# ChalmersPhotonicsLab/QAMpy

Hardware: AMD Instinct MI355X
Metric: equalised MSym/s (2-pol, 2 SPS) (higher is better)
Workload: dtype f32

## Files before the change

### qampy_amd/csrc/api.hip

```cpp
#include "common.h"
#include <stdlib.h>
#include <atomic>
#include <mutex>
#include <vector>
#include <unordered_map>
#include <string.h>

namespace qh {

thread_local hipStream_t g_stream = nullptr;
static thread_local hipStream_t g_streams[4] = {nullptr, nullptr, nullptr, nullptr};
int g_device = -1;
static thread_local std::string g_err;
static std::mutex g_mu;

void set_error(const std::string &s) { g_err = s; }

int hip_fail(hipError_t e, const char *what, const char *file, int line)
{
    g_err = std::string(hipGetErrorString(e)) + " in " + what + " (" + file + ":" + std::to_string(line) + ")";
    (void)hipGetLastError();
    return QH_ERR_HIP;
}

// ... 71 lines not shown
hipStream_t helper_stream() { return g_streams[3]; }

int ensure_init()
{
    if (g_stream) return QH_OK;
    return init_device(g_device >= 0 ? g_device : 0);
}

thread_local void *g_scratch[SCRATCH_SLOTS] = {nullptr};
thread_local size_t g_scratch_n[SCRATCH_SLOTS] = {0};
thread_local unsigned g_scratch_epoch = 0;
static std::atomic<int> g_form[FORM_COUNT];
struct FormName { const char *key, *env; };
static const FormName FORM_NAMES[FORM_COUNT] = {
    {"trainer", "QAMPY_HIP_TRAINER"}, {"pit_form", "QAMPY_HIP_PIT_FORM"}, {"seg_lanes", "QAMPY_HIP_SEG_LANES"}, {"pit_probe", "QAMPY_HIP_PIT_PROBE"},
    {"bps", "QAMPY_HIP_BPS"}, {"pit_tail", "QAMPY_HIP_PIT_TAIL"}};
static int form_parse(int k, const char *v, int *out)
{
    if (!v || !v[0]) { *out = 0; return 0; }
    switch (k) {
    case FORM_TRAINER: *out = v[0] == 'd' ? 1 : (v[0] == 'l' ? 2 : (v[0] == 'i' ? 3 : (v[0] == 'a' || v[0] == '0' ? 0 : -1))); break;
    case FORM_PIT: *out = v[0] == 's' ? 1 : (v[0] == 'b' ? 2 : (v[0] == 'a' || v[0] == '0' ? 0 : -1)); break;
    case FORM_SEG_LANES: { const int n = atoi(v); *out = (n == 8 || n == 16 || n == 0) ? n : -1; break; }
    case FORM_BPS: *out = v[0] == 't' ? 1 : (v[0] == 'l' ? 2 : (v[0] == 'a' || v[0] == '0' ? 0 : -1)); break;
    case FORM_PIT_TAIL: *out = v[0] == 's' ? 1 : (v[0] == 'a' || v[0] == '0' ? 0 : -1); break;
    default: *out = atoi(v) != 0 ? 1 : 0; break;
    }
    return *out < 0 ? -1 : 0;
}
static const int g_form_env_read = [] {
    for (int k = 0; k < FORM_COUNT; k++) {
        int v = 0;
        if (form_parse(k, getenv(FORM_NAMES[k].env), &v) == 0) g_form[k].store(v);
    }
    return 0;
}();
int form(FormKey k) { return g_form[k].load(std::memory_order_relaxed); }
const char *trainer_force()
{
    switch (form(FORM_TRAINER)) {
// ... 378 lines not shown
```

### qampy_amd/csrc/common.h

```cpp
#pragma once
#include <hip/hip_runtime.h>
#include <stdint.h>
#include <string>
#include "../../include/qampy_hip.h"

namespace qh {

extern thread_local hipStream_t g_stream;
extern int g_device;
void set_error(const std::string &s);
int hip_fail(hipError_t e, const char *what, const char *file, int line);

#define QH_HIP(call)                                                        \
    do {                                                                    \
        hipError_t _e = (call);                                             \
        if (_e != hipSuccess) return qh::hip_fail(_e, #call, __FILE__, __LINE__); \
    } while (0)

#define QH_REQUIRE(cond, msg)                                   \
    do {                                                        \
        if (!(cond)) { qh::set_error(msg); return QH_ERR_ARG; } \
    } while (0)

#define QH_WAVE_FIRST() __builtin_amdgcn_s_setprio(3)

int ensure_init();
hipStream_t side_stream();
hipStream_t helper_stream();
enum FormKey { FORM_TRAINER = 0, FORM_PIT, FORM_SEG_LANES, FORM_PIT_PROBE, FORM_BPS, FORM_PIT_TAIL, FORM_COUNT };
int form(FormKey k);
const char *trainer_force();
double gram_budget_gb();
int pit_timing_mode();
int default_tier();
double default_tier_tol();
constexpr int SCRATCH_SLOTS = 28;
constexpr int SCRATCH_TWOSTAGE = 16;
constexpr int SCRATCH_FOE = 17;
constexpr int SCRATCH_IMPAIR = 18;
constexpr int SCRATCH_PMD = 19;
constexpr int SCRATCH_TXRESP = 20;
constexpr int SCRATCH_SOS = 21;
constexpr int SCRATCH_CPR = 22;
constexpr int SCRATCH_FFT = 23;
// ... 173 lines not shown
```

### qampy_amd/csrc/train_pit.h

```cpp
#pragma once
#include <atomic>
#include <chrono>
#include <vector>
#include "train_impl.h"
#include "train_seg.h"

namespace qh {

typedef qh_pit_report PitCtrl;

constexpr double PIT_CONTRACT = 0.2;
constexpr int PIT_PROBE = 128;
constexpr int PIT_SEEDWIN = 512;
constexpr int PIT_MAXSEG = 65536;

__host__ __device__ inline int pit_symmetry(int method)
{
    switch (method) {
    case QH_M_CMA: case QH_M_SGNCMA: case QH_M_RDE: return 0;
    case QH_M_CMA2: return 2;
    default: return 4;
    }
}

// ... 34 lines not shown
    __syncthreads();
    return r;
}

template <typename T> __device__ __forceinline__ void block_prefix_sum(T *a, int n, T *tot)
{
    const int len = (n + 255) / 256;
    const int i0 = threadIdx.x * len, i1 = i0 + len < n ? i0 + len : n;
    T s = 0;
    for (int i = i0; i < i1; i++) s += a[i];
    T run = block_scan_excl<T>(s, [](T x, T y) { return x + y; }, (T)0, tot);
    for (int i = i0; i < i1; i++) { run += a[i]; a[i] = run; }
    __syncthreads();
}

template <typename R>
__global__ void __launch_bounds__(256) pit_setup_kernel(const Cx<R> *E, int nmodes, int64_t L, int64_t npow, int ntot, const R *mu, double gear,
                                                        double bound, double tol, PitSeg sg, PitCtrl *c, R *mu_acq)
{
    QH_WAVE_FIRST();
    __shared__ double red[256];
    double acc = 0;
    for (int k = 0; k < nmodes; k++)
        for (int64_t i = threadIdx.x; i < npow; i += 256) {
            const Cx<R> v = E[(size_t)k * L + i];
            acc += (double)v.re * v.re + (double)v.im * v.im;
        }
    red[threadIdx.x] = acc;
    __syncthreads();
    for (int s = 128; s > 0; s >>= 1) {
        if (threadIdx.x < s) red[threadIdx.x] += red[threadIdx.x + s];
        __syncthreads();
    }
    if (threadIdx.x == 0) {
        const double p = red[0] / ((double)nmodes * (double)npow);
        const double m = (double)*mu;
        double ma = gear * m;
        const double cap = bound / ((double)ntot * (p > 1e-30 ? p : 1e-30));
        if (ma > cap) ma = cap;
        if (!(ma > m)) ma = m;
        c->segments = sg.S; c->seg_len = sg.len; c->mu = m; c->mu_acq = ma; c->power = p; c->tol = tol;
        for (int q = 0; q < QH_PIT_MAXPASS; q++) { c->result_change[q] = -1; c->deviation[q] = -1; c->deviation_rms[q] = -1; c->deviation_taps[q] = -1; c->deviation_taps_worst[q] = -1; } c->passes = 0; c->converged = 0; c->acq_chunks = 0; c->acq_steps = 0; c->acq_done = 0; c->done = 0; c->diverged = 0; c->corr_on = 0; c->gain = 0; c->out_power = 0;
        for (int i = 0; i < QH_PIT_MAXPASS; i++) c->defect[i] = -1;
        for (int i = 0; i < QH_PIT_MAXCHUNK; i++) c->acq_err[i] = -1;
        *mu_acq = (R)ma;
    }
}

template <typename R>
__global__ void __launch_bounds__(256) pit_acq_monitor_kernel(const Cx<R> *err, int64_t err_pitch, int64_t step0, int64_t n, int nsel,
                                                              const int64_t *modes_dev, double plateau, PitCtrl *c, R *mu_acq, const R *mu, double floor_gear)
{
    QH_WAVE_FIRST();
    if (threadIdx.x == 0 && floor_gear >= 0) {
        const R lo = (R)((double)*mu * floor_gear), h = *mu_acq * (R)0.5;
        *mu_acq = h > lo ? h : (*mu_acq > lo ? lo : *mu_acq);
    }
    if (c->acq_done) return;
    __shared__ double red[256];
    double acc = 0;
// ... 72 lines not shown
            }
        }
        const double y2r = (double)yr * yr - (double)yi * yi, y2i = 2.0 * yr * yi;
        zr += y2r * y2r - y2i * y2i;
        zi += 2.0 * y2r * y2i;
    }
    rr[threadIdx.x] = zr; ri[threadIdx.x] = zi;
    __syncthreads();
    for (int q = 128; q > 0; q >>= 1) {
        if (threadIdx.x < q) { rr[threadIdx.x] += rr[threadIdx.x + q]; ri[threadIdx.x] += ri[threadIdx.x + q]; }
        __syncthreads();
    }
    if (threadIdx.x == 0) { z[2 * ((size_t)s * gridDim.y + j)] = rr[0]; z[2 * ((size_t)s * gridDim.y + j) + 1] = ri[0]; }
}

static __global__ void __launch_bounds__(256) pit_unwrap_kernel(const double *z, int S, int nsel, double *rot, double *phi, int *jump)
{
    QH_WAVE_FIRST();
    __shared__ int ptot[512];
    const double q = 1.5707963267948966;
    phi += (size_t)blockIdx.x * S; jump += (size_t)blockIdx.x * S;
    for (int j = blockIdx.x; j <= (int)blockIdx.x; j++) {
        for (int s = threadIdx.x; s < S; s += 256) {
            const double zr = z[2 * ((size_t)s * nsel + j)], zi = z[2 * ((size_t)s * nsel + j) + 1];
            phi[s] = (zr == 0 && zi == 0) ? 0.0 : (double)atan2f((float)-zi, (float)-zr) / 4;
        }
        __syncthreads();
        for (int s = threadIdx.x; s < S; s += 256) jump[s] = s == 0 ? 0 : (int)rint((phi[s - 1] - phi[s]) / q);
        __syncthreads();
        block_prefix_sum<int>(jump, S, ptot);
        for (int s = threadIdx.x; s < S; s += 256) {
            const double p = phi[s] + q * (jump[s] & 3);
            float sn, cs;
            sincosf((float)p, &sn, &cs);
            rot[2 * ((size_t)s * nsel + j)] = cs;
            rot[2 * ((size_t)s * nsel + j) + 1] = -sn;
        }
        __syncthreads();
    }
}

template <typename R>
__global__ void __launch_bounds__(256) pit_seed_kernel(const Cx<R> *wx, int nmodes, int ntot, const int64_t *modes_dev, int nsel, const double *rot, Cx<R> *X,
                                                       const Cx<R> *w0, Cx<R> *Y, PitCtrl *c)
{
    QH_WAVE_FIRST();
    const int s = blockIdx.x;
    const int n = nmodes * ntot;
    if (s == 0 && c) {
        if (threadIdx.x == 0) { c->done = 0; c->converged = 0; c->passes = 0; }
        for (int q = threadIdx.x; q < QH_PIT_MAXPASS; q += 256) {
            c->result_change[q] = -1; c->deviation[q] = -1; c->deviation_rms[q] = -1; c->deviation_taps[q] = -1; c->deviation_taps_worst[q] = -1; c->defect[q] = -1;
        }
    }
    const bool exact0 = s == 0 && w0 != nullptr;
    for (int e = threadIdx.x; e < n; e += 256) {
        const int row = e / ntot;
        Cx<R> v = exact0 ? w0[e] : wx[e];
        if (rot && !exact0) {
            for (int j = 0; j < nsel; j++)
                if ((int)modes_dev[j] == row) {
                    const double c = rot[2 * ((size_t)s * nsel + j)], d = rot[2 * ((size_t)s * nsel + j) + 1];
                    const double vr = (double)v.re * c - (double)v.im * d, vi = (double)v.re * d + (double)v.im * c;
                    v = Cx<R>{(R)vr, (R)vi};
                    break;
                }
        }
        X[(size_t)s * n + e] = v;
        Y[(size_t)s * n + e] = v;
    }
}

template <typename R>
__global__ void __launch_bounds__(PIT_PROBE) pit_defect_kernel(const Cx<R> *E, int nmodes, int64_t L, int os, int ntaps, PitSeg sg, int64_t TrSyms,
                                                                const int64_t *modes_dev, const Cx<R> *X, const Cx<R> *Y, int sym, const PitCtrl *c, double *dfc, double *pw, double *gph,
                                                                const Cx<R> *wx_prev)
{
// ... 1341 lines not shown
            const float nw = pass == 0 ? (float)run : old + relax * ((float)run - old);
            const float rel = fabsf(nw - old) / (fabsf(old) > 1e-30f ? fabsf(old) : 1e-30f);
            worst = (rel > worst || !(rel == rel)) ? (rel == rel ? rel : 3.0e38f) : worst;
            rS[s] = (R)nw;
            eS[s] = eE[s - 1];
        }
        run = A * run + B;
    }
    for (int o = 32; o > 0; o >>= 1) { const float w2 = __shfl_xor(worst, o); worst = worst > w2 ? worst : w2; }
    if ((threadIdx.x & 63) == 0) red[threadIdx.x >> 6] = worst;
    __syncthreads();
    if (threadIdx.x == 0) { float m = 0.f; for (int w = 0; w < 16; w++) m = m > red[w] ? m : red[w]; chg[0] = m; }
}
template <typename R> __global__ void pit_adapt_finish_kernel(R *mu, const R *rE, int n) { *mu = (R)1 / rE[n - 1]; }

struct PitInit { void *z[3]; unsigned zn[3]; void *cd[2]; const void *cs[2]; unsigned cn[2]; int64_t *modes_dev; int64_t modes[16]; int nsel; };
static __global__ void __launch_bounds__(256) pit_init_kernel(PitInit a)
{
    QH_WAVE_FIRST();
    const unsigned t = blockIdx.x * 256 + threadIdx.x, nt = gridDim.x * 256;
#pragma unroll
    for (int r = 0; r < 3; r++)
        if (a.z[r]) for (unsigned i = t; i < a.zn[r] / 4; i += nt) reinterpret_cast<uint32_t *>(a.z[r])[i] = 0u;
#pragma unroll
    for (int r = 0; r < 2; r++)
        if (a.cd[r]) for (unsigned i = t; i < a.cn[r] / 8; i += nt) reinterpret_cast<uint64_t *>(a.cd[r])[i] = reinterpret_cast<const uint64_t *>(a.cs[r])[i];
    if ((int)t < a.nsel) a.modes_dev[t] = a.modes[t];
}
constexpr int PIT_GT_THREADS = 1024;
template <typename R>
__global__ void __launch_bounds__(PIT_GT_THREADS) pit_gauge_kernel(const double *gph, int S, int nsel, PitCtrl *c, double *theta, const double *pw, int nb, int method, const Cx<R> *sy0,
                                                                   int want_corr, const PitModel *model = nullptr, const float4 *ualpha = nullptr, float2 *uq = nullptr,
                                                                   const R *mu = nullptr, int64_t T = 0, const float *Msum = nullptr)
{
    QH_WAVE_FIRST();
    if (c->done) return;
    constexpr int NT = PIT_GT_THREADS;
    __shared__ double redp[NT / 64];
    __shared__ double2 gbuf[NT / 64];
    __shared__ float4 abuf[NT / 64];
    if (gridDim.x > 1 && blockIdx.x == 1 && !(model && uq)) return;
    if (model && uq && (gridDim.x == 1 || blockIdx.x == 1)) {
        const bool corr = c->passes == 0 ? true : c->corr_on != 0;
// ... 395 lines not shown
    QH_REQUIRE(sg.S >= 2, "pit prepare: not preparable (nothing to parallelise)");
    const char *not_prep = "pit prepare: not preparable (throughput-form passes, block-form acquisition, blind error function)";
    QH_REQUIRE(!(method == QH_M_SBD || method == QH_M_MDDMA || method == QH_M_DD || method == QH_M_SBD_DATA), not_prep);
    TrainerForm f;
    if ((rc = trainer_form<R>(f, FORM_PASSES, method, 0, nmodes, ntaps, os, sg.len, (int64_t)sg.S * nsel, symbols, nsy, modes, nsel))) return rc;
    QH_REQUIRE(f.seg && f.block && la_shape_ok(nmodes, ntaps, os), not_prep);
    const PitPrepLayout lay = pit_prep_layout<R>(nmodes, ntaps, pl.amax);
    QH_REQUIRE(prep_bytes >= lay.total, "pit prepare: preparation buffer too small (qh_pit_prepare_bytes)");
    char *pb = (char *)prep;
    PitCtrl *ctrl = (PitCtrl *)(pb + lay.ctrl);
    R *mu_acq = (R *)(pb + lay.mu_acq);
    int64_t *modes_dev = (int64_t *)(pb + lay.modes);
    Cx<R> *wxp = (Cx<R> *)(pb + lay.wx), *w0 = (Cx<R> *)(pb + lay.w0), *errp = (Cx<R> *)(pb + lay.err);
    const size_t wset = (size_t)nmodes * ntot, wbytes = wset * sizeof(Cx<R>);
    const int64_t npow = L < 4096 ? L : 4096;
    hipLaunchKernelGGL((pit_setup_kernel<R>), dim3(1), dim3(256), 0, g_stream, (const Cx<R> *)E, nmodes, L, npow, ntot, mu_dev, pl.gear, pl.bound, o.tol > 0 ? o.tol : 1e-3, sg, ctrl, mu_acq);
    PitInit init{};
    init.cd[0] = wxp; init.cs[0] = wx0; init.cn[0] = (unsigned)wbytes;
    init.cd[1] = w0; init.cs[1] = wx0; init.cn[1] = (unsigned)wbytes;
    init.modes_dev = modes_dev; init.nsel = nsel;
    for (int j = 0; j < 16; j++) init.modes[j] = j < nsel ? modes[j] : 0;
    hipLaunchKernelGGL(pit_init_kernel, dim3(32), dim3(256), 0, g_stream, init);
    QH_REQUIRE(pl.ngram <= lay.err_pitch, "pit prepare: acquisition range exceeds the preparation buffer");
    void *G = nullptr;
    rc = f.pair_tab ? gram_build<R>(E, nmodes, L, os, ntaps, pl.ngram, &G, 1, 0, 0, pb + lay.gram) : QH_ERR_ARG;
    if (rc) return rc;
    LaArgs<R> la = la_args<R>(E, L, nmodes, ntaps, os, modes, nsel, method, symbols, nsy, mu_acq, errp, lay.err_pitch);
    la.G = (const GramPair<R> *)G; la.gpair = 1;
    if ((rc = pit_acq_enqueue<R>(pl, &la, f.use_bi, nullptr, wxp, errp, lay.err_pitch, ctrl, mu_acq, mu_dev, modes_dev, nsel))) return rc;
    hipLaunchKernelGGL((pit_acq_finish_kernel<R>), dim3((unsigned)((wset + 255) / 256)), dim3(256), 0, g_stream, wxp, (const Cx<R> *)w0, (int)wset, ctrl);
    QH_HIP(hipGetLastError());
// ... 22 lines not shown
    };
    QH_REQUIRE(o.segments >= 0 && o.segments <= PIT_MAXSEG && o.max_passes >= 0 && o.max_passes <= QH_PIT_MAXPASS, "train_equaliser: bad segment / pass count");
    QH_REQUIRE(o.adaptive >= 0 && o.adaptive <= 2, "train_equaliser: adaptive must be 0, 1 or 2");
    bool adaptive = o.adaptive != 0;
    {
        bool exact_only = method == QH_M_SBD_DATA;
        if (adaptive && (o.adaptive == 2 || sizeof(R) != 4 || nsel != 1 || Niter != 1 || !seg_adaptive_supported(method))) exact_only = true;
        QH_REQUIRE(!(adaptive && o.exchange), "train_equaliser: a capture split over processes is trained with a fixed step");
        if (exact_only) {
            QH_REQUIRE(!o.exchange, "train_equaliser: a capture split over processes needs the parallel-in-time solver (blind / decision-directed method, fixed step)");
            void *cb0 = nullptr;
            if ((rc = scratch(8, sizeof(PitCtrl) + 64, &cb0))) return rc;
            PitCtrl *c0 = report_dev ? (PitCtrl *)report_dev : (PitCtrl *)cb0;
            PitSeg s1; s1.S = 1; s1.len = TrSyms; s1.extra = 0; s1.tail = 0;
            hipLaunchKernelGGL((pit_setup_kernel<R>), dim3(1), dim3(256), 0, g_stream, (const Cx<R> *)E, nmodes, L, (int64_t)(L < 4096 ? L : 4096), nmodes * ntaps, (const R *)mu_dev, 1.0, 1.0,
                               o.tol > 0 ? o.tol : 1e-3, s1, c0, (R *)((char *)cb0 + sizeof(PitCtrl)));
            return exact_form(c0, o.adaptive, zero_err, adaptive ? nullptr : gram, 0);
        }
    }
    if (adaptive) o.acquire = 0;
    const int ntot = nmodes * ntaps;
    const int npass = o.max_passes > 0 ? o.max_passes : (adaptive ? QH_PIT_MAXPASS : 16);
    const double tol = (o.tol > 0 ? o.tol : 1e-3) * (adaptive ? 1.0 / 3.0 : 1.0);
    const double safety = o.dev_safety > 0 ? o.dev_safety : PIT_DEV_SAFETY;
    const int sym = pit_symmetry(method);
    const bool seed_phase = o.phase_seed < 0 ? sym == 4 : o.phase_seed != 0;
    const bool want_corr = o.correction != 0 && pit_basis_ok(ntot, sizeof(Cx<R>));
    double beta = o.corr_beta >= 0 ? o.corr_beta : (sym == 0 ? 1.5 : 0.0);

    void *cbuf = nullptr;
    if ((rc = scratch(8, sizeof(PitCtrl) + 64, &cbuf))) return rc;
// ... 17 lines not shown
        if (t > seg_want) seg_want = t;
    }
    if (S == 0 && adaptive) S = (int)((TrSyms - head) / seg_want < PIT_MAXSEG ? (TrSyms - head) / seg_want : PIT_MAXSEG);
    if (S == 0) {
        R mu_h = (R)o.mu_hint;
        if (!(o.mu_hint > 0)) {
            QH_HIP(hipMemcpyAsync(&mu_h, mu_dev, sizeof(R), hipMemcpyDeviceToHost, g_stream));
            QH_HIP(hipStreamSynchronize(g_stream));
        }
        S = pit_auto_segments(TrSyms, (double)mu_h, nsel, o.acquire);
    }
    PitPlan pl = pit_plan(o, TrSyms, head, S, adaptive, o.acquire ? o.acq_chunk : 0);
    const PitSeg &sg = pl.sg;
    if (zero_err) QH_HIP(hipMemsetAsync(err, 0, (size_t)nmodes * TrSyms * Niter * sizeof(Cx<R>), g_stream));
    const int64_t npow = L < 4096 ? L : 4096;
    hipLaunchKernelGGL((pit_setup_kernel<R>), dim3(1), dim3(256), 0, g_stream, (const Cx<R> *)E, nmodes, L, npow, ntot, (const R *)mu_dev, pl.gear, pl.bound, tol, sg, ctrl, mu_acq);
    QH_HIP(hipGetLastError());
    if (TrSyms == 0 || Niter == 0) return QH_OK;
    if (sg.S < 2) {
        const double zero = 0;
        QH_HIP(hipMemcpyAsync(&ctrl->defect[0], &zero, sizeof(double), hipMemcpyHostToDevice, g_stream));
        return exact_form(ctrl, adaptive ? 1 : 0, 0, gram, 1);
    }

    TrainerForm f;
    if ((rc = trainer_form<R>(f, FORM_PASSES, method, adaptive, nmodes, ntaps, os, sg.len, (int64_t)sg.S * nsel, symbols, nsy, modes, nsel))) return rc;
    if (adaptive && !f.seg) return exact_form(ctrl, 1, 0, nullptr, 0);
    const bool decision = method == QH_M_SBD || method == QH_M_MDDMA || method == QH_M_DD;
    const bool seg_form = f.seg, use_bi = f.use_bi, block_form = f.block, pair_tab = f.pair_tab;
    const bool split = o.exchange != nullptr;
    const int own_first = split ? o.seg_first : 0, own_count = split ? o.seg_count : sg.S;
// ... 26 lines not shown
    if (!adaptive && head > 0) {
        void *ab = nullptr;
        if ((rc = scratch(13, (size_t)nmodes * head * sizeof(Cx<R>) + 64, &ab))) return rc;
        ad_errh = (Cx<R> *)ab;
    }
    if (adaptive) {
        void *ab = nullptr;
        const size_t nS = ((size_t)sg.S + 15) / 16 * 16;
        if ((rc = scratch(13, nS * (2 * sizeof(R) + 2 * sizeof(Cx<R>) + 3 * sizeof(float)) + 64 + (size_t)nmodes * head * sizeof(Cx<R>), &ab))) return rc;
        ad_eS = (Cx<R> *)ab; ad_eE = ad_eS + nS; ad_errh = ad_eE + nS;
        ad_rS = (R *)(ad_errh + (size_t)nmodes * head); ad_rE = ad_rS + nS;
        ad_M = (float *)(ad_rE + nS); ad_rP = ad_M + nS; ad_dP = ad_rP + nS; ad_chg = ad_dP + nS;
    }
    init.modes_dev = modes_dev; init.nsel = nsel;
    for (int j = 0; j < 16; j++) init.modes[j] = j < nsel ? modes[j] : 0;
    const bool prepared = o.prepared != nullptr && o.acquire && !adaptive && head == 0 && Niter >= 1;
    const bool need_mu = adaptive || !(o.mu_hint > 0), need_acq = o.acquire && !(o.acq_chunk > 0) && !prepared;
    R mu_acq_h = 0;
    if (need_acq) QH_HIP(hipMemcpyAsync(&mu_acq_h, mu_acq, sizeof(R), hipMemcpyDeviceToHost, g_stream));
    R mu_host = need_mu ? (R)1 : (R)o.mu_hint;
    if (need_mu) QH_HIP(hipMemcpyAsync(&mu_host, mu_dev, sizeof(R), hipMemcpyDeviceToHost, g_stream));
    if (need_mu || need_acq) QH_HIP(hipStreamSynchronize(g_stream));
    if (!adaptive && !(mu_host != 0))
        return exact_form(ctrl, 0, 0, gram, 0);
    if (o.acquire && !(o.acq_chunk > 0)) pl.acquisition(o, TrSyms, pit_acq_chunk(mu_acq_h));

    const int64_t amax = pl.amax;
    void *G = const_cast<void *>(gram);
    if (prepared) QH_REQUIRE(seg_form && o.acq_chunk > 0, "train_equaliser: a prepared acquisition belongs to throughput-form passes with acq_chunk given (qh_pit_prepare_*_dev said so)");
    if (block_form && !G && (!seg_form || amax > 0) && !prepared) {
        const int64_t n = seg_form ? pl.ngram : TrSyms;
        rc = pair_tab ? gram_build<R>(E, nmodes, L, os, ntaps, n, &G) : gram_cur_build<R>(E, nmodes, L, os, ntaps, n, &G);
// ... 56 lines not shown
    LaArgs<R> la = la_args<R>(E, L, nmodes, ntaps, os, modes, nsel, method, symbols, nsy, mu_dev, err, TrSyms * Niter);
    la.G = (const GramPair<R> *)G; la.gpair = pair_tab ? 1 : 0; la.wx_cs = (int64_t)wset;
    la.dd_general = f.dd_general;
    f.alphabet(la);
    const TrainArgs<R> ta = train_args<R>(E, L, nmodes, ntaps, os, TrSyms, Niter, modes, nsel, method, symbols, nsy, mu_dev, err);

    PitTiming &tm = pit_timing();
    tm.npass = 0; tm.acq_ms = 0;
    bool acq_timed = false;
    PitEvents &ev = pit_events();
    QH_REQUIRE(ev.ok, "train_equaliser: no pinned memory for the pass flags");
    const bool redo_ok = o.exact_redo_off == 0;
    bool fell_back = false;
    if (redo_ok && !adaptive) { init.cd[0] = w_call; init.cs[0] = wx; init.cn[0] = (unsigned)wbytes; }
    if (o.acquire && Niter > 0) { init.cd[1] = w_start; init.cs[1] = wx; init.cn[1] = (unsigned)wbytes; }
    hipLaunchKernelGGL(pit_init_kernel, dim3(32), dim3(256), 0, g_stream, init);
    QH_HIP(hipGetLastError());
    for (int it = 0; it < Niter; it++) {
        if (it == 0 && prepared) {
            const PitPrepLayout lay = pit_prep_layout<R>(nmodes, ntaps, amax);
            const char *pb = (const char *)o.prepared;
            hipLaunchKernelGGL((pit_adopt_kernel<R>), dim3((unsigned)((wset + 255) / 256)), dim3(256), 0, g_stream, (Cx<R> *)wx, (const Cx<R> *)(pb + lay.wx), (int)wset,
                               (const PitCtrl *)(pb + lay.ctrl), ctrl, mu_acq, (const R *)(pb + lay.mu_acq));
            QH_HIP(hipGetLastError());
        } else if (it == 0 && o.acquire) {
            if (pl.nchunks > 0) { QH_HIP(hipEventRecord(ev.t0[PIT_NEV - 1], g_stream)); acq_timed = true; }
            if ((rc = pit_acq_enqueue<R>(pl, block_form ? &la : nullptr, use_bi, &ta, (Cx<R> *)wx, (Cx<R> *)err, TrSyms * Niter, ctrl, mu_acq, mu_dev,
                                         modes_dev, nsel))) return rc;
            if (pl.nchunks > 0) QH_HIP(hipEventRecord(ev.t1[PIT_NEV - 1], g_stream));
            hipLaunchKernelGGL((pit_acq_finish_kernel<R>), dim3((unsigned)((wset + 255) / 256)), dim3(256), 0, g_stream, (Cx<R> *)wx, (const Cx<R> *)w_start, (int)wset, ctrl);
            QH_HIP(hipGetLastError());
        }
        if (adaptive) {
            QH_HIP(hipMemcpyAsync(w_start, wx, wbytes, hipMemcpyDeviceToDevice, g_stream));
// ... 4 lines not shown
                               sg.S, ad_rS, ad_eS);
            QH_HIP(hipGetLastError());
        }
        if (!adaptive && head > 0) {
            if ((rc = train_dev<R>(E, nmodes, L, head, 1, os, mu_dev, wx, ntaps, modes, nsel, 0, symbols, nsy, method, ad_errh, 0, nullptr))) return rc;
            for (int j = 0; j < nsel; j++)
                QH_HIP(hipMemcpyAsync((Cx<R> *)err + (size_t)modes[j] * TrSyms * Niter + (size_t)it * TrSyms, ad_errh + (size_t)modes[j] * head, (size_t)head * sizeof(Cx<R>),
                                      hipMemcpyDeviceToDevice, g_stream));
        }
        const double *rot_use = nullptr;
        if (seed_phase) {
            int nwin = PIT_SEEDWIN;
            auto phase_lds = [&](int nw) { return ((size_t)ntot + (size_t)nmodes * os * pit_phase_pitch(ntaps, os, nw)) * sizeof(Cx<R>); };
            while (nwin > 32 && phase_lds(nwin) > 60 * 1024) nwin /= 2;
            QH_REQUIRE(phase_lds(nwin) <= 60 * 1024, "train_equaliser: phase seeding does not fit the LDS for this filter shape (pass phase_seed = 0)");
            hipLaunchKernelGGL((pit_phase_kernel<R>), dim3(sg.S, nsel), dim3(256), phase_lds(nwin), g_stream, (const Cx<R> *)E, nmodes, L, os,
                               (const Cx<R> *)wx, ntaps, sg, (const int64_t *)modes_dev, nwin, z);
            hipLaunchKernelGGL(pit_unwrap_kernel, dim3(nsel), dim3(256), 0, g_stream, (const double *)z, sg.S, nsel, rot, uw_phi, uw_jump);
            rot_use = rot;
        }
        const Cx<R> *w_exact = o.start == 1 ? nullptr : ((it == 0 && o.acquire) ? (const Cx<R> *)w_start : (const Cx<R> *)wx);
        hipLaunchKernelGGL((pit_seed_kernel<R>), dim3(sg.S), dim3(256), 0, g_stream, (const Cx<R> *)wx, nmodes, ntot, (const int64_t *)modes_dev, nsel, rot_use, X, w_exact, Y, ctrl);
        if (ssb) {
            ma.sg = sg; ma.rot = rot_use;
            static thread_local hipEvent_t ev_seed = nullptr, ev_model = nullptr;
            if (!ev_seed) { QH_HIP(hipEventCreateWithFlags(&ev_seed, hipEventDisableTiming)); QH_HIP(hipEventCreateWithFlags(&ev_model, hipEventDisableTiming)); }
            hipStream_t ss = helper_stream();
            QH_HIP(hipEventRecord(ev_seed, g_stream));
            QH_HIP(hipStreamWaitEvent(ss, ev_seed, 0));
            hipLaunchKernelGGL((pit_model_kernel<R, 0>), dim3(PIT_MODB), dim3(256), 0, ss, ma);
            hipLaunchKernelGGL((pit_model_kernel<R, 1>), dim3(PIT_MODB), dim3(256), 0, ss, ma);
            QH_HIP(hipEventRecord(ev_model, ss));
            model_event = ev_model;
        }
        QH_HIP(hipGetLastError());
        const int timing_mode = pit_timing_mode();
        auto decide_args = [&](int p, const float *dm, const float2 *ye, float2 *yprev, int ne, int ncol_e, int corr_wanted) {
            PitDecideArgs<R> d;
            d.dfc = dfc; d.pw = pw; d.nb = (int)((sg.S - 1) * nsel); d.Ylast = (const Cx<R> *)(Y + (size_t)(sg.S - 1) * wset); d.n = (int)wset; d.wx = (Cx<R> *)wx; d.c = ctrl;
            d.host_view = &ev.hview[2 * p]; d.nrow = nsel; d.devmax = dm; d.ndev = ndev; d.safety = safety; d.Ye = ye; d.Yprev = yprev; d.ne = ne; d.ncol_e = ncol_e;
            d.theta = theta; d.modes_dev = (const int64_t *)modes_dev; d.ntot_w = ntot; d.S = (int)sg.S; d.sym = sym; d.corr_wanted = corr_wanted;
            d.extra = adaptive ? (const float *)ad_chg : nullptr;
            d.Dfin = (ye && !adaptive) ? (const float2 *)Dz[1] : nullptr; d.Vfin = (const float2 *)Vb; d.lam_fin = lam;
            d.stall_from = o.correction == 0 ? QH_PIT_MAXPASS : (adaptive ? 5 : 2);
            return d;
        };
        auto timed = [&](int p) { return timing_mode == 2 || (timing_mode == 1 && p == 1); };
        int back_done_for = 0;
// ... 39 lines not shown
                ls.TrSyms = sg.len; ls.nch = sg.S; ls.wx = Y; ls.err_off = (int64_t)it * TrSyms; ls.seg = 1; ls.seg_extra = sg.extra; ls.seg_tail = sg.tail;
                ls.skip = &ctrl->done;
                pit_last_launch() = PitLaunch{use_bi ? 2 : 3, 0, 0, 0, 0, 0};
                if (sg.begin > 0) {
                    ls.E = (const Cx<R> *)E + sg.begin * os; ls.L = L - sg.begin * os; ls.err_off += sg.begin;
                    ls.G = (const GramPair<R> *)G + sg.begin * g_per_step;
                }
                { int r = use_bi ? launch_bi<R>(ls) : launch_la<R>(ls); if (r) return r; }
            } else {
                TrainArgs<R> ts = ta;
                ts.wx = Y; ts.nseg = sg.S; ts.seg_begin = sg.begin; ts.seg_len = sg.len; ts.seg_extra = sg.extra; ts.seg_tail = sg.tail; ts.seg_iter = it; ts.skip = &ctrl->done;
                pit_last_launch() = PitLaunch{4, 0, 0, 0, 0, 0};
                { int r = launch_any<R>(ts); if (r) return r; }
            }
            if (timed(p)) QH_HIP(hipEventRecord(ev.t1[p], g_stream));
            if (split) {
                if (own_first > 0) QH_HIP(hipMemsetAsync(Y, 0, (size_t)own_first * wbytes, g_stream));
                if (own_first + own_count < sg.S)
                    QH_HIP(hipMemsetAsync(Y + (size_t)(own_first + own_count) * wset, 0, (size_t)(sg.S - own_first - own_count) * wbytes, g_stream));
                if (!xchg_async) QH_HIP(hipStreamSynchronize(g_stream));
                if (o.exchange(o.exchange_user, Y, (size_t)sg.S * wbytes) != 0) { set_error("train_equaliser: the exchange callback failed"); return QH_ERR_ARG; }
            }
            const int nbnd = (int)((sg.S - 1) * nsel);
            if (eig) {
                if (o.basis && pit_basis_sync().pending) {
                    QH_HIP(hipStreamWaitEvent(g_stream, pit_basis_sync().out, 0));
                    pit_basis_sync().pending = false;
                }
                auto forward2 = [&](const Cx<R> *src, Zf *dst, const Cx<R> *src2, Zf *dst2) {
                    PitFuse<R> f2 = fz;
// ... 202 lines not shown
```

Measured before the change: 1241.

## Fuse PIT setup with init and adoption, merge phase and unwrap passes

Measured after the change: 1255 (median of 6 runs). +1.1%, better.

```diff
diff --git a/qampy_amd/csrc/api.hip b/qampy_amd/csrc/api.hip
--- a/qampy_amd/csrc/api.hip
+++ b/qampy_amd/csrc/api.hip
@@ -109,7 +109,7 @@
 struct FormName { const char *key, *env; };
 static const FormName FORM_NAMES[FORM_COUNT] = {
     {"trainer", "QAMPY_HIP_TRAINER"}, {"pit_form", "QAMPY_HIP_PIT_FORM"}, {"seg_lanes", "QAMPY_HIP_SEG_LANES"}, {"pit_probe", "QAMPY_HIP_PIT_PROBE"},
-    {"bps", "QAMPY_HIP_BPS"}, {"pit_tail", "QAMPY_HIP_PIT_TAIL"}};
+    {"bps", "QAMPY_HIP_BPS"}, {"pit_tail", "QAMPY_HIP_PIT_TAIL"}, {"pit_open", "QAMPY_HIP_PIT_OPEN"}};
 static int form_parse(int k, const char *v, int *out)
 {
     if (!v || !v[0]) { *out = 0; return 0; }
@@ -118,7 +118,7 @@
     case FORM_PIT: *out = v[0] == 's' ? 1 : (v[0] == 'b' ? 2 : (v[0] == 'a' || v[0] == '0' ? 0 : -1)); break;
     case FORM_SEG_LANES: { const int n = atoi(v); *out = (n == 8 || n == 16 || n == 0) ? n : -1; break; }
     case FORM_BPS: *out = v[0] == 't' ? 1 : (v[0] == 'l' ? 2 : (v[0] == 'a' || v[0] == '0' ? 0 : -1)); break;
-    case FORM_PIT_TAIL: *out = v[0] == 's' ? 1 : (v[0] == 'a' || v[0] == '0' ? 0 : -1); break;
+    case FORM_PIT_TAIL: case FORM_PIT_OPEN: *out = v[0] == 's' ? 1 : (v[0] == 'a' || v[0] == '0' ? 0 : -1); break;
     default: *out = atoi(v) != 0 ? 1 : 0; break;
     }
     return *out < 0 ? -1 : 0;
diff --git a/qampy_amd/csrc/common.h b/qampy_amd/csrc/common.h
--- a/qampy_amd/csrc/common.h
+++ b/qampy_amd/csrc/common.h
@@ -27,7 +27,7 @@
 int ensure_init();
 hipStream_t side_stream();
 hipStream_t helper_stream();
-enum FormKey { FORM_TRAINER = 0, FORM_PIT, FORM_SEG_LANES, FORM_PIT_PROBE, FORM_BPS, FORM_PIT_TAIL, FORM_COUNT };
+enum FormKey { FORM_TRAINER = 0, FORM_PIT, FORM_SEG_LANES, FORM_PIT_PROBE, FORM_BPS, FORM_PIT_TAIL, FORM_PIT_OPEN, FORM_COUNT };
 int form(FormKey k);
 const char *trainer_force();
 double gram_budget_gb();
diff --git a/qampy_amd/csrc/train_pit.h b/qampy_amd/csrc/train_pit.h
--- a/qampy_amd/csrc/train_pit.h
+++ b/qampy_amd/csrc/train_pit.h
@@ -72,11 +72,48 @@
     __syncthreads();
 }
 
+struct PitInit {
+    void *z[3]; unsigned zn[3]; void *cd[2]; const void *cs[2]; unsigned cn[2]; int64_t *modes_dev; int64_t modes[16]; int nsel;
+    void *wx; const void *wx_prep; void *w_call, *w_start; unsigned wn;
+    const PitCtrl *prep; const void *mu_acq_prep;
+};
+__device__ __forceinline__ void pit_init_body(const PitInit &a, unsigned t, unsigned nt)
+{
+#pragma unroll
+    for (int r = 0; r < 3; r++)
+        if (a.z[r]) for (unsigned i = t; i < a.zn[r] / 4; i += nt) reinterpret_cast<uint32_t *>(a.z[r])[i] = 0u;
+#pragma unroll
+    for (int r = 0; r < 2; r++)
+        if (a.cd[r]) for (unsigned i = t; i < a.cn[r] / 8; i += nt) reinterpret_cast<uint64_t *>(a.cd[r])[i] = reinterpret_cast<const uint64_t *>(a.cs[r])[i];
+    if (a.wx_prep) {
+        const bool keep = a.prep->diverged != 0;
+        uint64_t *w = reinterpret_cast<uint64_t *>(a.wx);
+        for (unsigned i = t; i < a.wn / 8; i += nt) {
+            const uint64_t v = w[i];
+            if (a.w_call) reinterpret_cast<uint64_t *>(a.w_call)[i] = v;
+            if (a.w_start) reinterpret_cast<uint64_t *>(a.w_start)[i] = v;
+            if (!keep) w[i] = reinterpret_cast<const uint64_t *>(a.wx_prep)[i];
+        }
+    }
+    if ((int)t < a.nsel) a.modes_dev[t] = a.modes[t];
+}
+static __global__ void __launch_bounds__(256) pit_init_kernel(PitInit a)
+{
+    QH_WAVE_FIRST();
+    pit_init_body(a, blockIdx.x * 256 + threadIdx.x, gridDim.x * 256);
+}
+
 template <typename R>
 __global__ void __launch_bounds__(256) pit_setup_kernel(const Cx<R> *E, int nmodes, int64_t L, int64_t npow, int ntot, const R *mu, double gear,
-                                                        double bound, double tol, PitSeg sg, PitCtrl *c, R *mu_acq)
+                                                        double bound, double tol, PitSeg sg, PitCtrl *c, R *mu_acq, PitInit init)
 {
     QH_WAVE_FIRST();
+    if (blockIdx.x > 0) { pit_init_body(init, (blockIdx.x - 1) * 256 + threadIdx.x, (gridDim.x - 1) * 256); return; }
+    const PitCtrl *prep = gridDim.x > 1 ? init.prep : nullptr;
+    for (int q = threadIdx.x; q < QH_PIT_MAXPASS; q += 256) {
+        c->result_change[q] = -1; c->deviation[q] = -1; c->deviation_rms[q] = -1; c->deviation_taps[q] = -1; c->deviation_taps_worst[q] = -1; c->defect[q] = -1;
+    }
+    for (int i = threadIdx.x; i < QH_PIT_MAXCHUNK; i += 256) c->acq_err[i] = prep ? prep->acq_err[i] : -1;
     __shared__ double red[256];
     double acc = 0;
     for (int k = 0; k < nmodes; k++)
@@ -98,10 +135,12 @@
         if (ma > cap) ma = cap;
         if (!(ma > m)) ma = m;
         c->segments = sg.S; c->seg_len = sg.len; c->mu = m; c->mu_acq = ma; c->power = p; c->tol = tol;
-        for (int q = 0; q < QH_PIT_MAXPASS; q++) { c->result_change[q] = -1; c->deviation[q] = -1; c->deviation_rms[q] = -1; c->deviation_taps[q] = -1; c->deviation_taps_worst[q] = -1; } c->passes = 0; c->converged = 0; c->acq_chunks = 0; c->acq_steps = 0; c->acq_done = 0; c->done = 0; c->diverged = 0; c->corr_on = 0; c->gain = 0; c->out_power = 0;
-        for (int i = 0; i < QH_PIT_MAXPASS; i++) c->defect[i] = -1;
-        for (int i = 0; i < QH_PIT_MAXCHUNK; i++) c->acq_err[i] = -1;
+        c->passes = 0; c->converged = 0; c->acq_chunks = 0; c->acq_steps = 0; c->acq_done = 0; c->done = 0; c->diverged = 0; c->corr_on = 0; c->gain = 0; c->out_power = 0;
         *mu_acq = (R)ma;
+        if (prep) {
+            c->acq_chunks = prep->acq_chunks; c->acq_steps = prep->acq_steps; c->acq_done = 1; c->diverged = prep->diverged; c->mu_acq = prep->mu_acq;
+            *mu_acq = *reinterpret_cast<const R *>(init.mu_acq_prep);
+        }
     }
 }
 
@@ -204,6 +243,87 @@
     if (threadIdx.x == 0) { z[2 * ((size_t)s * gridDim.y + j)] = rr[0]; z[2 * ((size_t)s * gridDim.y + j) + 1] = ri[0]; }
 }
 
+template <typename R, int MJ>
+__global__ void __launch_bounds__(256) pit_phase_all_kernel(const Cx<R> *__restrict__ E, int nmodes, int64_t L, int os, const Cx<R> *__restrict__ wx, int ntaps, PitSeg sg,
+                                                            const int64_t *__restrict__ modes_dev, int nsel, int nwin, double *__restrict__ z, double *__restrict__ phi)
+{
+    QH_WAVE_FIRST();
+    extern __shared__ __attribute__((aligned(16))) char pit_smem[];
+    Cx<R> *xs = reinterpret_cast<Cx<R> *>(pit_smem);
+    const int ntot = nmodes * ntaps;
+    const int pitch = nwin + (ntaps + os - 1) / os + 1;
+    __shared__ double rr[256], ri[256];
+    const int s = blockIdx.x;
+    const int64_t st = sg.start(s);
+    int64_t n = sg.steps(s);
+    if (n > nwin) n = nwin;
+    const int ns = n > 0 ? (int)(n - 1) * os + ntaps : 0;
+    for (int k = 0; k < nmodes; k++) {
+        const Cx<R> *x = E + (size_t)k * L + st * os;
+        for (int g = threadIdx.x; g < ns; g += 256) xs[((size_t)k * os + g % os) * pitch + g / os] = x[g];
+    }
+    __syncthreads();
+    for (int j0 = 0; j0 < nsel; j0 += MJ) {
+        const Cx<R> *wj[MJ];
+#pragma unroll
+        for (int q = 0; q < MJ; q++) wj[q] = wx + (size_t)modes_dev[j0 + q < nsel ? j0 + q : nsel - 1] * ntot;
+        double zr[MJ], zi[MJ];
+#pragma unroll
+        for (int q = 0; q < MJ; q++) { zr[q] = 0; zi[q] = 0; }
+        for (int i = threadIdx.x; i < n; i += 512) {
+            const int second = i + 256 < n ? 256 : 0;
+            R yr[2][MJ], yi[2][MJ];
+#pragma unroll
+            for (int q = 0; q < MJ; q++) { yr[0][q] = 0; yi[0][q] = 0; yr[1][q] = 0; yi[1][q] = 0; }
+            for (int k = 0; k < nmodes; k++) {
+                for (int r = 0; r < os; r++) {
+                    const Cx<R> *xp = xs + ((size_t)k * os + r) * pitch + i;
+                    int u = 0;
+#pragma unroll 4
+                    for (int t = r; t < ntaps; t += os, u++) {
+                        const Cx<R> a0 = xp[u], a1 = xp[u + second];
+#pragma unroll
+                        for (int q = 0; q < MJ; q++) {
+                            const Cx<R> b = wj[q][k * ntaps + t];
+                            yr[0][q] = fma_(a0.re, b.re, fma_(-a0.im, b.im, yr[0][q]));
+                            yi[0][q] = fma_(a0.re, b.im, fma_(a0.im, b.re, yi[0][q]));
+                            yr[1][q] = fma_(a1.re, b.re, fma_(-a1.im, b.im, yr[1][q]));
+                            yi[1][q] = fma_(a1.re, b.im, fma_(a1.im, b.re, yi[1][q]));
+                        }
+                    }
+                }
+            }
+#pragma unroll
+            for (int o = 0; o < 2; o++) {
+                if (o == 1 && !second) break;
+#pragma unroll
+                for (int q = 0; q < MJ; q++) {
+                    const double y2r = (double)yr[o][q] * yr[o][q] - (double)yi[o][q] * yi[o][q], y2i = 2.0 * yr[o][q] * yi[o][q];
+                    zr[q] += y2r * y2r - y2i * y2i;
+                    zi[q] += 2.0 * y2r * y2i;
+                }
+            }
+        }
+#pragma unroll
+        for (int q = 0; q < MJ; q++) {
+            if (j0 + q >= nsel) break;
+            rr[threadIdx.x] = zr[q]; ri[threadIdx.x] = zi[q];
+            __syncthreads();
+            for (int h = 128; h > 0; h >>= 1) {
+                if (threadIdx.x < h) { rr[threadIdx.x] += rr[threadIdx.x + h]; ri[threadIdx.x] += ri[threadIdx.x + h]; }
+                __syncthreads();
+            }
+            if (threadIdx.x == 0) {
+                const int j = j0 + q;
+                const double vr = rr[0], vi = ri[0];
+                z[2 * ((size_t)s * nsel + j)] = vr; z[2 * ((size_t)s * nsel + j) + 1] = vi;
+                phi[(size_t)j * sg.S + s] = (vr == 0 && vi == 0) ? 0.0 : (double)atan2f((float)-vi, (float)-vr) / 4;
+            }
+            __syncthreads();
+        }
+    }
+}
+
 static __global__ void __launch_bounds__(256) pit_unwrap_kernel(const double *z, int S, int nsel, double *rot, double *phi, int *jump)
 {
     QH_WAVE_FIRST();
@@ -232,11 +352,36 @@
 
 template <typename R>
 __global__ void __launch_bounds__(256) pit_seed_kernel(const Cx<R> *wx, int nmodes, int ntot, const int64_t *modes_dev, int nsel, const double *rot, Cx<R> *X,
-                                                       const Cx<R> *w0, Cx<R> *Y, PitCtrl *c)
+                                                       const Cx<R> *w0, Cx<R> *Y, PitCtrl *c, const double *phi = nullptr, double *rot_out = nullptr)
 {
     QH_WAVE_FIRST();
     const int s = blockIdx.x;
     const int n = nmodes * ntot;
+    __shared__ int wsum[16][4];
+    __shared__ double own[16][2];
+    if (phi) {
+        const double q = 1.5707963267948966;
+        const int S = gridDim.x, lane = threadIdx.x & 63, wave = threadIdx.x >> 6;
+        for (int j = 0; j < nsel; j++) {
+            const double *pj = phi + (size_t)j * S;
+            int acc = 0;
+            for (int k = 1 + threadIdx.x; k <= s; k += 256) acc += (int)rint((pj[k - 1] - pj[k]) / q);
+            for (int o = 32; o > 0; o >>= 1) acc += __shfl_xor(acc, o);
+            if (lane == 0) wsum[j][wave] = acc;
+        }
+        __syncthreads();
+        if ((int)threadIdx.x < nsel) {
+            const int j = threadIdx.x;
+            const int jump = wsum[j][0] + wsum[j][1] + wsum[j][2] + wsum[j][3];
+            const double p = phi[(size_t)j * S + s] + q * (jump & 3);
+            float sn, cs;
+            sincosf((float)p, &sn, &cs);
+            own[j][0] = cs; own[j][1] = -sn;
+            rot_out[2 * ((size_t)s * nsel + j)] = cs;
+            rot_out[2 * ((size_t)s * nsel + j) + 1] = -sn;
+        }
+        __syncthreads();
+    }
     if (s == 0 && c) {
         if (threadIdx.x == 0) { c->done = 0; c->converged = 0; c->passes = 0; }
         for (int q = threadIdx.x; q < QH_PIT_MAXPASS; q += 256) {
@@ -247,10 +392,10 @@
     for (int e = threadIdx.x; e < n; e += 256) {
         const int row = e / ntot;
         Cx<R> v = exact0 ? w0[e] : wx[e];
-        if (rot && !exact0) {
+        if ((rot || phi) && !exact0) {
             for (int j = 0; j < nsel; j++)
                 if ((int)modes_dev[j] == row) {
-                    const double c = rot[2 * ((size_t)s * nsel + j)], d = rot[2 * ((size_t)s * nsel + j) + 1];
+                    const double c = phi ? own[j][0] : rot[2 * ((size_t)s * nsel + j)], d = phi ? own[j][1] : rot[2 * ((size_t)s * nsel + j) + 1];
                     const double vr = (double)v.re * c - (double)v.im * d, vi = (double)v.re * d + (double)v.im * c;
                     v = Cx<R>{(R)vr, (R)vi};
                     break;
@@ -1622,19 +1767,6 @@
 }
 template <typename R> __global__ void pit_adapt_finish_kernel(R *mu, const R *rE, int n) { *mu = (R)1 / rE[n - 1]; }
 
-struct PitInit { void *z[3]; unsigned zn[3]; void *cd[2]; const void *cs[2]; unsigned cn[2]; int64_t *modes_dev; int64_t modes[16]; int nsel; };
-static __global__ void __launch_bounds__(256) pit_init_kernel(PitInit a)
-{
-    QH_WAVE_FIRST();
-    const unsigned t = blockIdx.x * 256 + threadIdx.x, nt = gridDim.x * 256;
-#pragma unroll
-    for (int r = 0; r < 3; r++)
-        if (a.z[r]) for (unsigned i = t; i < a.zn[r] / 4; i += nt) reinterpret_cast<uint32_t *>(a.z[r])[i] = 0u;
-#pragma unroll
-    for (int r = 0; r < 2; r++)
-        if (a.cd[r]) for (unsigned i = t; i < a.cn[r] / 8; i += nt) reinterpret_cast<uint64_t *>(a.cd[r])[i] = reinterpret_cast<const uint64_t *>(a.cs[r])[i];
-    if ((int)t < a.nsel) a.modes_dev[t] = a.modes[t];
-}
 constexpr int PIT_GT_THREADS = 1024;
 template <typename R>
 __global__ void __launch_bounds__(PIT_GT_THREADS) pit_gauge_kernel(const double *gph, int S, int nsel, PitCtrl *c, double *theta, const double *pw, int nb, int method, const Cx<R> *sy0,
@@ -2060,7 +2192,7 @@
     Cx<R> *wxp = (Cx<R> *)(pb + lay.wx), *w0 = (Cx<R> *)(pb + lay.w0), *errp = (Cx<R> *)(pb + lay.err);
     const size_t wset = (size_t)nmodes * ntot, wbytes = wset * sizeof(Cx<R>);
     const int64_t npow = L < 4096 ? L : 4096;
-    hipLaunchKernelGGL((pit_setup_kernel<R>), dim3(1), dim3(256), 0, g_stream, (const Cx<R> *)E, nmodes, L, npow, ntot, mu_dev, pl.gear, pl.bound, o.tol > 0 ? o.tol : 1e-3, sg, ctrl, mu_acq);
+    hipLaunchKernelGGL((pit_setup_kernel<R>), dim3(1), dim3(256), 0, g_stream, (const Cx<R> *)E, nmodes, L, npow, ntot, mu_dev, pl.gear, pl.bound, o.tol > 0 ? o.tol : 1e-3, sg, ctrl, mu_acq, PitInit{});
     PitInit init{};
     init.cd[0] = wxp; init.cs[0] = wx0; init.cn[0] = (unsigned)wbytes;
     init.cd[1] = w0; init.cs[1] = wx0; init.cn[1] = (unsigned)wbytes;
@@ -2113,7 +2245,7 @@
             PitCtrl *c0 = report_dev ? (PitCtrl *)report_dev : (PitCtrl *)cb0;
             PitSeg s1; s1.S = 1; s1.len = TrSyms; s1.extra = 0; s1.tail = 0;
             hipLaunchKernelGGL((pit_setup_kernel<R>), dim3(1), dim3(256), 0, g_stream, (const Cx<R> *)E, nmodes, L, (int64_t)(L < 4096 ? L : 4096), nmodes * ntaps, (const R *)mu_dev, 1.0, 1.0,
-                               o.tol > 0 ? o.tol : 1e-3, s1, c0, (R *)((char *)cb0 + sizeof(PitCtrl)));
+                               o.tol > 0 ? o.tol : 1e-3, s1, c0, (R *)((char *)cb0 + sizeof(PitCtrl)), PitInit{});
             return exact_form(c0, o.adaptive, zero_err, adaptive ? nullptr : gram, 0);
         }
     }
@@ -2161,7 +2293,18 @@
     const PitSeg &sg = pl.sg;
     if (zero_err) QH_HIP(hipMemsetAsync(err, 0, (size_t)nmodes * TrSyms * Niter * sizeof(Cx<R>), g_stream));
     const int64_t npow = L < 4096 ? L : 4096;
-    hipLaunchKernelGGL((pit_setup_kernel<R>), dim3(1), dim3(256), 0, g_stream, (const Cx<R> *)E, nmodes, L, npow, ntot, (const R *)mu_dev, pl.gear, pl.bound, tol, sg, ctrl, mu_acq);
+    const bool open_auto = form(FORM_PIT_OPEN) == 0;
+    const bool prepared = o.prepared != nullptr && o.acquire && !adaptive && head == 0 && Niter >= 1;
+    const bool need_mu = adaptive || !(o.mu_hint > 0), need_acq = o.acquire && !(o.acq_chunk > 0) && !prepared;
+    auto setup_alone = [&]() {
+        hipLaunchKernelGGL((pit_setup_kernel<R>), dim3(1), dim3(256), 0, g_stream, (const Cx<R> *)E, nmodes, L, npow, ntot, (const R *)mu_dev, pl.gear, pl.bound, tol, sg, ctrl, mu_acq,
+                           PitInit{});
+    };
+    struct SetupOwed {
+        decltype(setup_alone) &pay; bool owed;
+        ~SetupOwed() { if (owed) pay(); }
+    } setup_owed{setup_alone, open_auto && !need_mu && !need_acq && TrSyms > 0 && Niter > 0 && sg.S >= 2};
+    if (!setup_owed.owed) setup_alone();
     QH_HIP(hipGetLastError());
     if (TrSyms == 0 || Niter == 0) return QH_OK;
     if (sg.S < 2) {
@@ -2218,8 +2361,6 @@
     }
     init.modes_dev = modes_dev; init.nsel = nsel;
     for (int j = 0; j < 16; j++) init.modes[j] = j < nsel ? modes[j] : 0;
-    const bool prepared = o.prepared != nullptr && o.acquire && !adaptive && head == 0 && Niter >= 1;
-    const bool need_mu = adaptive || !(o.mu_hint > 0), need_acq = o.acquire && !(o.acq_chunk > 0) && !prepared;
     R mu_acq_h = 0;
     if (need_acq) QH_HIP(hipMemcpyAsync(&mu_acq_h, mu_acq, sizeof(R), hipMemcpyDeviceToHost, g_stream));
     R mu_host = need_mu ? (R)1 : (R)o.mu_hint;
@@ -2306,10 +2447,25 @@
     bool fell_back = false;
     if (redo_ok && !adaptive) { init.cd[0] = w_call; init.cs[0] = wx; init.cn[0] = (unsigned)wbytes; }
     if (o.acquire && Niter > 0) { init.cd[1] = w_start; init.cs[1] = wx; init.cn[1] = (unsigned)wbytes; }
-    hipLaunchKernelGGL(pit_init_kernel, dim3(32), dim3(256), 0, g_stream, init);
+    const bool adopt_merged = setup_owed.owed && prepared;
+    if (adopt_merged) {
+        const PitPrepLayout lay = pit_prep_layout<R>(nmodes, ntaps, amax);
+        const char *pb = (const char *)o.prepared;
+        init.wx = wx; init.wx_prep = pb + lay.wx; init.wn = (unsigned)wbytes;
+        init.w_call = init.cd[0]; init.w_start = init.cd[1];
+        init.cd[0] = nullptr; init.cd[1] = nullptr;
+        init.prep = (const PitCtrl *)(pb + lay.ctrl); init.mu_acq_prep = pb + lay.mu_acq;
+    }
+    if (setup_owed.owed) {
+        setup_owed.owed = false;
+        hipLaunchKernelGGL((pit_setup_kernel<R>), dim3(1 + 32), dim3(256), 0, g_stream, (const Cx<R> *)E, nmodes, L, npow, ntot, (const R *)mu_dev, pl.gear, pl.bound, tol, sg, ctrl, mu_acq,
+                           init);
+    } else
+        hipLaunchKernelGGL(pit_init_kernel, dim3(32), dim3(256), 0, g_stream, init);
     QH_HIP(hipGetLastError());
     for (int it = 0; it < Niter; it++) {
-        if (it == 0 && prepared) {
+        if (it == 0 && adopt_merged) {
+        } else if (it == 0 && prepared) {
             const PitPrepLayout lay = pit_prep_layout<R>(nmodes, ntaps, amax);
             const char *pb = (const char *)o.prepared;
             hipLaunchKernelGGL((pit_adopt_kernel<R>), dim3((unsigned)((wset + 255) / 256)), dim3(256), 0, g_stream, (Cx<R> *)wx, (const Cx<R> *)(pb + lay.wx), (int)wset,
@@ -2344,24 +2500,43 @@
             auto phase_lds = [&](int nw) { return ((size_t)ntot + (size_t)nmodes * os * pit_phase_pitch(ntaps, os, nw)) * sizeof(Cx<R>); };
             while (nwin > 32 && phase_lds(nwin) > 60 * 1024) nwin /= 2;
             QH_REQUIRE(phase_lds(nwin) <= 60 * 1024, "train_equaliser: phase seeding does not fit the LDS for this filter shape (pass phase_seed = 0)");
-            hipLaunchKernelGGL((pit_phase_kernel<R>), dim3(sg.S, nsel), dim3(256), phase_lds(nwin), g_stream, (const Cx<R> *)E, nmodes, L, os,
-                               (const Cx<R> *)wx, ntaps, sg, (const int64_t *)modes_dev, nwin, z);
-            hipLaunchKernelGGL(pit_unwrap_kernel, dim3(nsel), dim3(256), 0, g_stream, (const double *)z, sg.S, nsel, rot, uw_phi, uw_jump);
+            if (open_auto) {
+                const size_t lds = (size_t)nmodes * os * pit_phase_pitch(ntaps, os, nwin) * sizeof(Cx<R>);
+                auto launch_phase = [&](auto kern) {
+                    hipLaunchKernelGGL(kern, dim3(sg.S), dim3(256), lds, g_stream, (const Cx<R> *)E, nmodes, L, os, (const Cx<R> *)wx, ntaps, sg, (const int64_t *)modes_dev, nsel,
+                                       nwin, z, uw_phi);
+                };
+                if (nsel >= 4) launch_phase(pit_phase_all_kernel<R, 4>);
+                else if (nsel >= 2) launch_phase(pit_phase_all_kernel<R, 2>);
+                else launch_phase(pit_phase_all_kernel<R, 1>);
+            } else {
+                hipLaunchKernelGGL((pit_phase_kernel<R>), dim3(sg.S, nsel), dim3(256), phase_lds(nwin), g_stream, (const Cx<R> *)E, nmodes, L, os,
+                                   (const Cx<R> *)wx, ntaps, sg, (const int64_t *)modes_dev, nwin, z);
+                hipLaunchKernelGGL(pit_unwrap_kernel, dim3(nsel), dim3(256), 0, g_stream, (const double *)z, sg.S, nsel, rot, uw_phi, uw_jump);
+            }
             rot_use = rot;
         }
         const Cx<R> *w_exact = o.start == 1 ? nullptr : ((it == 0 && o.acquire) ? (const Cx<R> *)w_start : (const Cx<R> *)wx);
-        hipLaunchKernelGGL((pit_seed_kernel<R>), dim3(sg.S), dim3(256), 0, g_stream, (const Cx<R> *)wx, nmodes, ntot, (const int64_t *)modes_dev, nsel, rot_use, X, w_exact, Y, ctrl);
-        if (ssb) {
-            ma.sg = sg; ma.rot = rot_use;
-            static thread_local hipEvent_t ev_seed = nullptr, ev_model = nullptr;
-            if (!ev_seed) { QH_HIP(hipEventCreateWithFlags(&ev_seed, hipEventDisableTiming)); QH_HIP(hipEventCreateWithFlags(&ev_model, hipEventDisableTiming)); }
+        const bool seed_unwraps = seed_phase && open_auto;
+        hipLaunchKernelGGL((pit_seed_kernel<R>), dim3(sg.S), dim3(256), 0, g_stream, (const Cx<R> *)wx, nmodes, ntot, (const int64_t *)modes_dev, nsel,
+                           seed_unwraps ? (const double *)nullptr : rot_use, X, w_exact, Y, ctrl, seed_unwraps ? (const double *)uw_phi : (const double *)nullptr, rot);
+        static thread_local hipEvent_t ev_seed = nullptr, ev_model = nullptr;
+        auto enqueue_model = [&]() -> int {
             hipStream_t ss = helper_stream();
-            QH_HIP(hipEventRecord(ev_seed, g_stream));
             QH_HIP(hipStreamWaitEvent(ss, ev_seed, 0));
             hipLaunchKernelGGL((pit_model_kernel<R, 0>), dim3(PIT_MODB), dim3(256), 0, ss, ma);
             hipLaunchKernelGGL((pit_model_kernel<R, 1>), dim3(PIT_MODB), dim3(256), 0, ss, ma);
             QH_HIP(hipEventRecord(ev_model, ss));
+            return QH_OK;
+        };
+        bool model_late = false;
+        if (ssb) {
+            ma.sg = sg; ma.rot = rot_use;
+            if (!ev_seed) { QH_HIP(hipEventCreateWithFlags(&ev_seed, hipEventDisableTiming)); QH_HIP(hipEventCreateWithFlags(&ev_model, hipEventDisableTiming)); }
+            QH_HIP(hipEventRecord(ev_seed, g_stream));
             model_event = ev_model;
+            if (open_auto) model_late = true;
+            else if ((rc = enqueue_model())) return rc;
         }
         QH_HIP(hipGetLastError());
         const int timing_mode = pit_timing_mode();
@@ -2431,6 +2606,10 @@
                 { int r = launch_any<R>(ts); if (r) return r; }
             }
             if (timed(p)) QH_HIP(hipEventRecord(ev.t1[p], g_stream));
+            if (model_late) {
+                model_late = false;
+                if (int r = enqueue_model()) return r;
+            }
             if (split) {
                 if (own_first > 0) QH_HIP(hipMemsetAsync(Y, 0, (size_t)own_first * wbytes, g_stream));
                 if (own_first + own_count < sg.S)
```
